# DevSinghSachan/emdr2

Measured on AMD Instinct MI355X. Metric: mips_queries_per_sec, higher is better.
Workload: dtype f16; 1 GPU; BASELINE configs[1]: MIPS-only top-50, 512 queries/search over a 21015324 x 768 fp16 index resident in HBM; rows=21015324, dim=768, top_k=50, parallelism=index row-sharded x1, all-gather(top-k) + merge, cus=256, allgather_bytes_per_rank=0

## Files before the change

### emdr2_amd/csrc/mips_api.hip

```cpp
#include "../../include/emdr2_mips.h"
#include "mips_kernels.h"
#include "exp_hooks.h"
#include <stdlib.h>

namespace {

#define TIMING_SLOTS 2048
struct Timing {
    bool enabled = false;
    hipEvent_t ev[2 * TIMING_SLOTS] = {};
    int created = 0;
    int n = 0;
    int64_t rows[TIMING_SLOTS] = {};
} g_timing;

int cu_count()
{
    static int cus = 0;
    if (!cus) {
        int dev = 0;
        hipDeviceProp_t prop;
        if (hipGetDevice(&dev) != hipSuccess || hipGetDeviceProperties(&prop, dev) != hipSuccess) return 256;
        cus = prop.multiProcessorCount > 0 ? prop.multiProcessorCount : 256;
    }
    return cus;
}

inline size_t align_up(size_t x, size_t a) { return (x + a - 1) / a * a; }

#define env_int(name, dflt) EXP_ENV_INT(name, dflt)

struct Workspace {
    char *q_frag;
    char *q_tiled;
    float *qnorm, *tau;
    unsigned *count;
    uint2 *cand, *cand8;
};

size_t carve(char *base, int dim, Workspace *w)
{
    size_t off = 0;
    auto take = [&](size_t bytes) { char *p = base ? base + off : nullptr; off += align_up(bytes, 256); return p; };
    char *f = take((size_t)(dim / 32) * 512 * 64);
    char *a = take((size_t)(dim / 32) * 512 * 64);
    char *b = take(512 * sizeof(float));
    char *c = take(512 * sizeof(float));
    char *d = take((512 + 8 * 512 + 8 * (size_t)SCAN8_PROG_UINTS) * sizeof(unsigned));
    char *e = take((size_t)512 * CAPQ * sizeof(uint2));
    char *g = take((size_t)512 * 8 * SUBCAP * sizeof(uint2));
    if (w) { w->q_frag = f; w->q_tiled = a; w->qnorm = (float *)b; w->tau = (float *)c; w->count = (unsigned *)d; w->cand = (uint2 *)e; w->cand8 = (uint2 *)g; }
    return off;
}

struct Shadow {
    const void *image;
    const float *table;
    int64_t min_rows;
};
long g_shadow_launches = 0;

bool bad_shape(int64_t n_rows, int dim) { return n_rows < 0 || n_rows >= ((int64_t)1 << 31) - 1024 || dim < 64 || dim > 8192 || (dim % 32) != 0; }

}

extern "C" {

int emdr2_abi_version(void) { return EMDR2_ABI_VERSION; }

int emdr2_device_cu_count(void) { return cu_count(); }

int emdr2_mips_set_timing(int enabled)
{
    g_timing.enabled = enabled != 0;
    g_timing.n = 0;
    return EMDR2_OK;
}

int emdr2_mips_timing_collect(float *ms, int64_t *rows, int max_n, int *n_out)
{
    const int n = g_timing.n < max_n ? g_timing.n : max_n;
    for (int i = 0; i < n; ++i) {
        if (hipEventSynchronize(g_timing.ev[2 * i + 1]) != hipSuccess) return EMDR2_E_LAUNCH;
        if (hipEventElapsedTime(&ms[i], g_timing.ev[2 * i], g_timing.ev[2 * i + 1]) != hipSuccess) return EMDR2_E_LAUNCH;
        rows[i] = g_timing.rows[i];
    }
    if (n_out) *n_out = n;
    g_timing.n = 0;
    return EMDR2_OK;
}

int emdr2_mips_layout_bytes(int64_t n_rows, int dim, size_t *bytes)
{
    if (!bytes || bad_shape(n_rows, dim)) return EMDR2_E_BADARG;
    const int64_t padded = (n_rows + 511) / 512 * 512;
    *bytes = (size_t)padded * dim * 2;
    return EMDR2_OK;
}

int emdr2_mips_pack_rows(const void *rows_rm, int64_t n_chunk, int dim, int64_t row_offset, int64_t n_rows_total,
                         void *tiled, float *emax_sq, emdr2_stream_t stream)
{
    if (!rows_rm || !tiled || !emax_sq || bad_shape(n_rows_total, dim) || n_chunk < 0 || row_offset < 0 ||
        row_offset + n_chunk > n_rows_total)
        return EMDR2_E_BADARG;
    return mips_launch_pack_rows(rows_rm, n_chunk, dim, row_offset, tiled, emax_sq, (hipStream_t)stream);
}

int emdr2_mips_unpack_rows(const void *tiled, int64_t n_rows_total, int dim, const int64_t *row_ids, int64_t n_out,
                           void *rows_rm, emdr2_stream_t stream)
{
    if (!tiled || !row_ids || !rows_rm || bad_shape(n_rows_total, dim) || n_out < 0) return EMDR2_E_BADARG;
    return mips_launch_unpack_rows(tiled, dim, row_ids, n_out, rows_rm, (hipStream_t)stream);
}

int emdr2_mips_workspace_bytes(int n_q, int dim, int k, size_t *bytes)
{
    if (!bytes || n_q < 1 || k < 1 || k > EMDR2_MAX_TOPK || bad_shape(0, dim)) return EMDR2_E_BADARG;
    *bytes = carve(nullptr, dim, nullptr);
    return EMDR2_OK;
}

static int variant_for(int nq) { return nq <= 128 ? 2 : (nq <= 256 ? 1 : 0); }
static const int kBM[3] = {128, 256, 512};
static const int kBN[3] = {512, 256, 128};

static int search_impl(const void *tiled, int64_t n_rows, int dim, int64_t row_base, const float *emax_sq,
                       const void *queries, int n_q, int k, const int32_t *ids, void *out_dist, int32_t *out_idx,
                       int64_t *out_row, uint32_t *out_flags, void *workspace, size_t workspace_bytes,
                       emdr2_stream_t stream_, int f32, uint4 *out_rec = nullptr, const Shadow *shadow = nullptr)
{
    if (!tiled || !emax_sq || !queries || !out_flags || !workspace) return EMDR2_E_BADARG;
    if (!out_rec && (!out_dist || !out_idx || !out_row)) return EMDR2_E_BADARG;
    if (out_rec && ((uintptr_t)out_rec & 15)) return EMDR2_E_BADARG;
    if (n_q < 1 || k < 1 || k > EMDR2_MAX_TOPK || bad_shape(n_rows, dim) || n_rows < 1) return EMDR2_E_BADARG;
    Workspace w;
    if (carve((char *)workspace, dim, &w) > workspace_bytes) return EMDR2_E_WORKSPACE;
    hipStream_t stream = (hipStream_t)stream_;
    const int kp = k <= 56 ? 64 : 128;
    const int seg0 = env_int("EMDR2_MIPS_SEG0", 8192) / 512 * 512;
    const int growth = env_int("EMDR2_MIPS_GROWTH", 8);
    const int growth_i8 = env_int("EMDR2_MIPS_GROWTH_I8", 2);
    if (seg0 < 512 || seg0 > (int)CAPQ - 512 || growth < 2 || growth_i8 < 2) return EMDR2_E_BADARG;
    const int force_variant = env_int("EMDR2_MIPS_VARIANT", -1);
    const int cus = env_int("EMDR2_MIPS_GRID", cu_count());
    const int scan_kernel = env_int("EMDR2_MIPS_KERNEL", 1);
    const int ablate = env_int("EMDR2_MIPS_ABLATE", 0);

    for (int q0 = 0; q0 < n_q; q0 += EMDR2_MAX_QUERIES_PER_PASS) {
        const int nqp = (n_q - q0) < EMDR2_MAX_QUERIES_PER_PASS ? (n_q - q0) : EMDR2_MAX_QUERIES_PER_PASS;
        int variant = variant_for(nqp);
        if (force_variant >= 0 && force_variant <= 2 && kBN[force_variant] >= nqp) variant = force_variant;
        const int BM = kBM[variant], BN = kBN[variant];
        const uint16_t *qp = (const uint16_t *)queries + (size_t)q0 * dim;
        int rc;
        if ((rc = mips_launch_pack_queries(qp, nqp, dim, BN, w.q_tiled, w.qnorm, stream))) return rc;
        EXP_MIPS_PACK_QUERIES_FRAG(variant, scan_kernel, qp, nqp, dim, w, stream, rc)
        const int64_t dense_rows = n_rows < seg0 ? n_rows : seg0;
        unsigned *const count8 = w.count + 512, *const prog0 = count8 + 8 * 512;
        if ((rc = mips_launch_init(w.tau, w.count, out_flags + q0, BN, nqp, (unsigned)dense_rows, count8,
                                   8 * 512 + (variant == 0 ? 8 * (size_t)SCAN8_PROG_UINTS : 0), stream)))
            return rc;

        ScanParams sp;
        sp.e_tiled = (const char *)tiled;
        sp.q_tiled = w.q_tiled;
        sp.tau = w.tau;
        sp.cand = w.cand;
        sp.count = w.count;
        sp.flags = out_flags + q0;
        sp.dense_out = nullptr;
        sp.nch = dim / 32;
        sp.n_rows = (int)n_rows;
        sp.n_q = nqp;
        sp.capq = CAPQ;
        sp.cand8 = w.cand8;
        sp.count8 = count8;
        sp.dense_row0 = 0;
        sp.tune = env_int("EMDR2_MIPS_TUNE", 17);
        sp.trace = (unsigned long long *)w.cand + (size_t)511 * CAPQ;

        int scan8_launches = 0;
        const bool shadow_ok = shadow && variant <= 1 && scan_kernel == 1 && (dim % 256) == 0 && n_rows - dense_rows >= shadow->min_rows;
        char *const q8_tiled = w.q_frag;
        float *const qc = (float *)(w.q_frag + (size_t)(dim / 64) * 512 * 64);
        if (shadow_ok && (rc = mips_launch_pack_queries_i8(qp, nqp, dim, BN, q8_tiled, qc, stream))) return rc;
        const bool couple = EXP_MIPS_COUPLE();
        int64_t done = 0, seg_end = dense_rows;
        int mode = 1;
        while (done < n_rows) {
            sp.tile_begin = (int)(done / BM);
            sp.tile_end = (int)((seg_end + BM - 1) / BM);
            const int tiles = sp.tile_end - sp.tile_begin;
            const int grid = tiles < cus ? tiles : cus;
            const bool timed = g_timing.enabled && g_timing.n < TIMING_SLOTS;
            if (timed) {
                while (g_timing.created <= g_timing.n) {
                    if (hipEventCreate(&g_timing.ev[2 * g_timing.created]) != hipSuccess ||
                        hipEventCreate(&g_timing.ev[2 * g_timing.created + 1]) != hipSuccess)
                        return EMDR2_E_LAUNCH;
                    ++g_timing.created;
                }
                if (hipEventRecord(g_timing.ev[2 * g_timing.n], stream) != hipSuccess) return EMDR2_E_LAUNCH;
            }
            bool int8_segment = false;
            EXP_MIPS_SCAN_VARIANT(mode, variant, ablate, scan_kernel, sp, w, grid, seg_end, n_rows, done, stream, rc)
            {
                rc = -4;
                if (mode == 0 && variant <= 1 && scan_kernel == 1) {
                    unsigned *prog = (couple && scan8_launches < 8) ? prog0 + (size_t)SCAN8_PROG_UINTS * scan8_launches : nullptr;
                    if (shadow_ok && seg_end - done >= shadow->min_rows) {
                        rc = mips_launch_scan8i(sp, shadow->image, shadow->table, q8_tiled, qc, BN, done, seg_end, cus, prog, stream);
                        if (rc == 0) { int8_segment = true; ++g_shadow_launches; }
                    }
                    if (rc == -4) rc = mips_launch_scan8(sp, BN, done, seg_end, cus, prog, stream);
                    if (rc == 0) ++scan8_launches;
                }
                if (rc == -4) rc = mips_launch_scan(variant, mode, sp, grid, stream);
            }
            if (rc) return rc;
            if (timed) {
                if (hipEventRecord(g_timing.ev[2 * g_timing.n + 1], stream) != hipSuccess) return EMDR2_E_LAUNCH;
                g_timing.rows[g_timing.n] = seg_end - done;
                ++g_timing.n;
            }
            if (int8_segment && (rc = mips_launch_rescore(sp, qp, (unsigned)kp, stream))) return rc;
            if (seg_end < n_rows && (rc = mips_launch_select(w.cand, w.count, w.cand8, count8, w.tau, out_flags + q0, CAPQ, kp, nqp, stream))) return rc;
            done = seg_end;
            const int64_t next_boundary = done * ((shadow_ok && done * (growth_i8 - 1) >= shadow->min_rows) ? growth_i8 : growth);
            seg_end = next_boundary < n_rows ? next_boundary : n_rows;
            if (n_rows - seg_end < seg_end / 2) seg_end = n_rows;
            mode = 0;
        }

        FinalizeParams fp;
        fp.e_tiled = (const char *)tiled;
        fp.queries = qp;
        fp.cand = w.cand;
        fp.count = w.count;
        fp.cand8 = w.cand8;
        fp.count8 = count8;
        fp.tau = w.tau;
        fp.qnorm = w.qnorm;
        fp.emax_sq = emax_sq;
        fp.ids = ids;
        fp.out_rec = out_rec ? out_rec + (size_t)q0 * k : nullptr;
        fp.out_dist = out_rec ? nullptr : (f32 ? (void *)((float *)out_dist + (size_t)q0 * k) : (void *)((uint16_t *)out_dist + (size_t)q0 * k));
        fp.f32 = f32;
        fp.out_idx = out_rec ? nullptr : out_idx + (size_t)q0 * k;
        fp.out_row = out_rec ? nullptr : out_row + (size_t)q0 * k;
        fp.flags = out_flags + q0;
        fp.n_rows = n_rows;
        fp.row_base = row_base;
        fp.dim = dim;
        fp.n_q = nqp;
        fp.k = k;
        fp.kp = kp;
        fp.capq = CAPQ;
        if ((rc = mips_launch_finalize(fp, true, stream))) return rc;
    }
    return EMDR2_OK;
}

int emdr2_mips_search(const void *tiled, int64_t n_rows, int dim, int64_t row_base, const float *emax_sq,
                      const void *queries, int n_q, int k, const int32_t *ids, void *out_dist, int32_t *out_idx,
                      int64_t *out_row, uint32_t *out_flags, void *workspace, size_t workspace_bytes,
                      emdr2_stream_t stream)
{
    return search_impl(tiled, n_rows, dim, row_base, emax_sq, queries, n_q, k, ids, out_dist, out_idx, out_row, out_flags, workspace,
                       workspace_bytes, stream, 0);
}

int emdr2_mips_search_f32(const void *tiled, int64_t n_rows, int dim, int64_t row_base, const float *emax_sq,
                          const void *queries, int n_q, int k, const int32_t *ids, float *out_dist, int32_t *out_idx,
                          int64_t *out_row, uint32_t *out_flags, void *workspace, size_t workspace_bytes,
                          emdr2_stream_t stream)
{
    return search_impl(tiled, n_rows, dim, row_base, emax_sq, queries, n_q, k, ids, out_dist, out_idx, out_row, out_flags, workspace,
                       workspace_bytes, stream, 1);
}

int emdr2_mips_search_records(const void *tiled, int64_t n_rows, int dim, int64_t row_base, const float *emax_sq, const void *queries, int n_q,
                              int k, const int32_t *ids, int f32, void *out_records, uint32_t *out_flags, void *workspace,
                              size_t workspace_bytes, emdr2_stream_t stream)
{
    if (!out_records) return EMDR2_E_BADARG;
    return search_impl(tiled, n_rows, dim, row_base, emax_sq, queries, n_q, k, ids, nullptr, nullptr, nullptr, out_flags, workspace,
                       workspace_bytes, stream, f32 ? 1 : 0, (uint4 *)out_records);
}

int emdr2_mips_shadow_bytes(int64_t n_rows, int dim, size_t *image_bytes, size_t *table_bytes)
{
    if (!image_bytes || !table_bytes || bad_shape(n_rows, dim) || (dim % 256) != 0) return EMDR2_E_BADARG;
    const int64_t padded = (n_rows + 511) / 512 * 512;
    *image_bytes = (size_t)padded * dim;
    *table_bytes = (size_t)(padded / 256) * 4 * sizeof(float);
    return EMDR2_OK;
}

int emdr2_mips_seal_shadow(const void *tiled, int64_t n_rows, int dim, void *shadow, void *table, uint32_t *nonfinite, emdr2_stream_t stream)
{
    if (!tiled || !shadow || !table || !nonfinite || ((uintptr_t)table & 15) || bad_shape(n_rows, dim) || (dim % 256) != 0) return EMDR2_E_BADARG;
    return mips_launch_seal_shadow(tiled, n_rows, dim, shadow, (float *)table, nonfinite, (hipStream_t)stream);
}

int emdr2_mips_search_shadow(const void *tiled, int64_t n_rows, int dim, int64_t row_base, const float *emax_sq, const void *shadow,
                             const void *table, int64_t shadow_min_rows, const void *queries, int n_q, int k, const int32_t *ids, int f32,
                             void *out_dist, int32_t *out_idx, int64_t *out_row, void *out_records, uint32_t *out_flags, void *workspace,
                             size_t workspace_bytes, emdr2_stream_t stream)
{
    if (!shadow || !table || ((uintptr_t)table & 15) || shadow_min_rows < 1 || (dim % 256) != 0) return EMDR2_E_BADARG;
    const Shadow sh = {shadow, (const float *)table, shadow_min_rows};
    return search_impl(tiled, n_rows, dim, row_base, emax_sq, queries, n_q, k, ids, out_dist, out_idx, out_row, out_flags, workspace,
                       workspace_bytes, stream, f32 ? 1 : 0, (uint4 *)out_records, &sh);
}

int emdr2_mips_shadow_launches(void) { return (int)g_shadow_launches; }

int emdr2_mips_merge_records(const void *records_in, int n_shards, int n_q, int k, int f32, void *out_dist, int32_t *out_idx, int64_t *out_row,
                             emdr2_stream_t stream)
{
    if (!records_in || ((uintptr_t)records_in & 15) || !out_dist || !out_idx || !out_row || n_shards < 1 || n_q < 1 || k < 1) return EMDR2_E_BADARG;
    return mips_launch_merge_records((const uint4 *)records_in, n_shards, n_q, k, f32 ? 1 : 0, out_dist, out_idx, out_row, (hipStream_t)stream);
}

int emdr2_mips_pack_records(const void *dist, const int32_t *idx, const int64_t *row, const int32_t *sel, int n_sel, int k, int f32,
                            void *records, emdr2_stream_t stream)
{
    if (!dist || !idx || !row || !sel || !records || ((uintptr_t)records & 15) || n_sel < 0 || k < 1) return EMDR2_E_BADARG;
    return mips_launch_pack_records(dist, idx, row, sel, n_sel, k, f32 ? 1 : 0, (uint4 *)records, (hipStream_t)stream);
}

int emdr2_mips_exact_workspace_bytes_f32(int64_t n_rows, int n_sel, size_t *bytes)
{
    if (!bytes || n_rows < 1 || n_sel < 0) return EMDR2_E_BADARG;
    *bytes = align_up((size_t)8 * (size_t)n_rows * sizeof(uint32_t), 256);
    return EMDR2_OK;
}

int emdr2_mips_search_exact_f32(const void *tiled, int64_t n_rows, int dim, int64_t row_base, const void *queries,
                                int n_q, const int32_t *sel, int n_sel, int k, const int32_t *ids, float *out_dist,
                                int32_t *out_idx, int64_t *out_row, uint32_t *out_flags, void *workspace,
                                size_t workspace_bytes, emdr2_stream_t stream_)
{
    if (!tiled || !queries || !sel || !out_dist || !out_idx || !out_row || !out_flags || !workspace) return EMDR2_E_BADARG;
    if (n_q < 1 || n_sel < 0 || k < 1 || k > EMDR2_MAX_TOPK || bad_shape(n_rows, dim) || n_rows < 1) return EMDR2_E_BADARG;
    if (workspace_bytes < (size_t)8 * (size_t)n_rows * sizeof(uint32_t)) return EMDR2_E_WORKSPACE;
    hipStream_t stream = (hipStream_t)stream_;
    for (int b = 0; b < n_sel; b += 8) {
        const int nb = (n_sel - b) < 8 ? (n_sel - b) : 8;
        int rc;
        if ((rc = mips_launch_exact_scores_f32((const char *)tiled, n_rows, dim, (const uint16_t *)queries, sel + b, nb,
                                               (uint32_t *)workspace, stream)))
            return rc;
        if ((rc = mips_launch_exact_select_f32((const uint32_t *)workspace, n_rows, row_base, sel + b, nb, k, ids, out_dist, out_idx,
                                               out_row, out_flags, stream)))
            return rc;
    }
    return EMDR2_OK;
}

int emdr2_mips_merge_f32(const float *dist_in, const int32_t *idx_in, const int64_t *row_in, int n_shards, int n_q, int k,
                         float *out_dist, int32_t *out_idx, int64_t *out_row, emdr2_stream_t stream)
{
    if (!dist_in || !idx_in || !row_in || !out_dist || !out_idx || !out_row || n_shards < 1 || n_q < 1 || k < 1) return EMDR2_E_BADARG;
    return mips_launch_merge_f32(dist_in, idx_in, row_in, n_shards, n_q, k, out_dist, out_idx, out_row, (hipStream_t)stream);
}

int emdr2_mips_exact_workspace_bytes(int64_t n_rows, int n_sel, size_t *bytes)
{
    if (!bytes || n_rows < 1 || n_sel < 0) return EMDR2_E_BADARG;
    *bytes = align_up((size_t)8 * (size_t)n_rows * sizeof(uint16_t), 256);
    return EMDR2_OK;
}

int emdr2_mips_search_exact(const void *tiled, int64_t n_rows, int dim, int64_t row_base, const void *queries,
                            int n_q, const int32_t *sel, int n_sel, int k, const int32_t *ids, void *out_dist,
                            int32_t *out_idx, int64_t *out_row, uint32_t *out_flags, void *workspace,
                            size_t workspace_bytes, emdr2_stream_t stream_)
{
    if (!tiled || !queries || !sel || !out_dist || !out_idx || !out_row || !out_flags || !workspace) return EMDR2_E_BADARG;
    if (n_q < 1 || n_sel < 0 || k < 1 || k > EMDR2_MAX_TOPK || bad_shape(n_rows, dim) || n_rows < 1) return EMDR2_E_BADARG;
    if (workspace_bytes < (size_t)8 * (size_t)n_rows * sizeof(uint16_t)) return EMDR2_E_WORKSPACE;
    hipStream_t stream = (hipStream_t)stream_;
    for (int b = 0; b < n_sel; b += 8) {
        const int nb = (n_sel - b) < 8 ? (n_sel - b) : 8;
        int rc;
        if ((rc = mips_launch_exact_scores((const char *)tiled, n_rows, dim, (const uint16_t *)queries, sel + b, nb,
                                           (uint16_t *)workspace, stream)))
            return rc;
        if ((rc = mips_launch_exact_select((const uint16_t *)workspace, n_rows, row_base, sel + b, nb, k, ids,
                                           (uint16_t *)out_dist, out_idx, out_row, out_flags, stream)))
            return rc;
    }
    return EMDR2_OK;
}

int emdr2_mips_merge(const void *dist_in, const int32_t *idx_in, const int64_t *row_in, int n_shards, int n_q, int k,
                     void *out_dist, int32_t *out_idx, int64_t *out_row, emdr2_stream_t stream)
{
    if (!dist_in || !idx_in || !row_in || !out_dist || !out_idx || !out_row || n_shards < 1 || n_q < 1 || k < 1) return EMDR2_E_BADARG;
    return mips_launch_merge((const uint16_t *)dist_in, idx_in, row_in, n_shards, n_q, k, (uint16_t *)out_dist, out_idx,
                             out_row, (hipStream_t)stream);
}

int emdr2_mips_debug_scores(const void *tiled, int64_t n_rows, int dim, const void *queries, int n_q,
                            float *out_scores, void *workspace, size_t workspace_bytes, emdr2_stream_t stream_)
{
    if (!tiled || !queries || !out_scores || !workspace || n_q < 1 || n_q > 512 || bad_shape(n_rows, dim) || n_rows < 1) return EMDR2_E_BADARG;
    Workspace w;
    if (carve((char *)workspace, dim, &w) > workspace_bytes) return EMDR2_E_WORKSPACE;
    hipStream_t stream = (hipStream_t)stream_;
    int variant = variant_for(n_q);
    const int force_variant = env_int("EMDR2_MIPS_VARIANT", -1);
    if (force_variant >= 0 && force_variant <= 2 && kBN[force_variant] >= n_q) variant = force_variant;
    const int BM = kBM[variant], BN = kBN[variant];
    int rc;
    if ((rc = mips_launch_pack_queries(queries, n_q, dim, BN, w.q_tiled, w.qnorm, stream))) return rc;
    ScanParams sp;
    sp.e_tiled = (const char *)tiled;
    sp.q_tiled = w.q_tiled;
    sp.tau = w.tau;
    sp.cand = w.cand;
    sp.count = w.count;
    sp.flags = nullptr;
    sp.dense_out = out_scores;
    sp.nch = dim / 32;
    sp.n_rows = (int)n_rows;
    sp.n_q = n_q;
    sp.capq = CAPQ;
    sp.cand8 = nullptr;
    sp.count8 = nullptr;
    sp.dense_row0 = 0;
    sp.tune = 1;
    sp.trace = nullptr;
    sp.tile_begin = 0;
    sp.tile_end = (int)((n_rows + BM - 1) / BM);
    const int cus = cu_count();
    return mips_launch_scan(variant, 2, sp, sp.tile_end < cus ? sp.tile_end : cus, stream);
}

}
```

### emdr2_amd/csrc/mips_kernels.h

```cpp
#pragma once
#include <hip/hip_runtime.h>
#include <stdint.h>

#define CAPQ 16384u
#define SUBCAP 1024u

struct ScanParams {
    const char *e_tiled;
    const char *q_tiled;
    const float *tau;
    uint2 *cand;
    unsigned *count;
    unsigned *flags;
    float *dense_out;
    int nch;
    int tile_begin, tile_end;
    int n_rows;
    int n_q;
    unsigned capq;
    uint2 *cand8;
    unsigned *count8;
    int dense_row0;
    int tune;
    unsigned long long *trace;
};

int mips_launch_scan(int variant, int mode, const ScanParams &p, int grid, hipStream_t stream);
#define SCAN8_PROG_UINTS (256 * 64)
int mips_launch_scan8(const ScanParams &p, int bn, int64_t row_begin, int64_t row_end, int cus, unsigned *prog, hipStream_t stream);
int mips_launch_seal_shadow(const void *tiled, int64_t n_rows, int dim, void *e8, float *blk, unsigned *nonfinite, hipStream_t stream);
int mips_launch_pack_queries_i8(const void *queries, int n_q, int dim, int bn, void *q8_tiled, float *qc, hipStream_t stream);
int mips_launch_scan8i(const ScanParams &p, const void *e8_tiled, const float *blk, const void *q8_tiled, const float *qc, int bn, int64_t row_begin,
                       int64_t row_end, int cus, unsigned *prog, hipStream_t stream);
int mips_launch_rescore(const ScanParams &p, const void *queries, unsigned pre, hipStream_t stream);
int mips_launch_scan_pp(int variant, int depth, const ScanParams &p, int grid, hipStream_t stream);
int mips_launch_scan_q8(int abl, const ScanParams &p, int grid, hipStream_t stream);
int mips_launch_pack_queries_frag(const void *queries, int n_q, int dim, void *q_frag, hipStream_t stream);
int mips_launch_scan_ablate(int abl, const ScanParams &p, int grid, hipStream_t stream);

int mips_launch_pack_rows(const void *rows_rm, int64_t n_chunk, int dim, int64_t row_offset, void *tiled,
                          float *emax_sq, hipStream_t stream);
int mips_launch_unpack_rows(const void *tiled, int dim, const int64_t *row_ids, int64_t n_out, void *rows_rm,
                            hipStream_t stream);
int mips_launch_pack_queries(const void *queries, int n_q, int dim, int bn, void *q_tiled, float *qnorm,
                             hipStream_t stream);
int mips_launch_init(float *tau, unsigned *count, unsigned *flags, int bn, int n_q, unsigned dense_count, unsigned *zero, size_t n_zero,
                     hipStream_t stream);
int mips_launch_select(uint2 *cand, unsigned *count, uint2 *cand8, unsigned *count8, float *tau, unsigned *flags, unsigned capq, int kp, int n_q,
                       hipStream_t stream);
struct FinalizeParams {
    const char *e_tiled;
    const uint16_t *queries;
    const uint2 *cand;
    const unsigned *count;
    uint2 *cand8;
    unsigned *count8;
    const float *tau;
    const float *qnorm;
    const float *emax_sq;
    const int32_t *ids;
    void *out_dist;
    int32_t *out_idx;
    int64_t *out_row;
    unsigned *flags;
    int64_t n_rows, row_base;
    int dim, n_q, k, kp;
    unsigned capq;
    int f32;
    uint4 *out_rec;
};
int mips_launch_finalize(const FinalizeParams &p, bool select_first, hipStream_t stream);
int mips_launch_merge_f32(const float *dist_in, const int32_t *idx_in, const int64_t *row_in, int n_shards, int n_q, int k,
                          float *out_dist, int32_t *out_idx, int64_t *out_row, hipStream_t stream);
int mips_launch_merge_records(const uint4 *rec_in, int n_shards, int n_q, int k, int f32, void *out_dist, int32_t *out_idx, int64_t *out_row,
                              hipStream_t stream);
int mips_launch_pack_records(const void *dist, const int32_t *idx, const int64_t *row, const int32_t *sel, int n_sel, int k, int f32, uint4 *rec,
                             hipStream_t stream);
int mips_launch_merge(const uint16_t *dist_in, const int32_t *idx_in, const int64_t *row_in, int n_shards, int n_q,
                      int k, uint16_t *out_dist, int32_t *out_idx, int64_t *out_row, hipStream_t stream);

int mips_launch_exact_scores(const char *e_tiled, int64_t n_rows, int dim, const uint16_t *queries,
                             const int32_t *sel, int n_sel, uint16_t *hkeys ,
                             hipStream_t stream);
int mips_launch_exact_select(const uint16_t *hkeys, int64_t n_rows, int64_t row_base, const int32_t *sel, int n_sel,
                             int k, const int32_t *ids, uint16_t *out_dist, int32_t *out_idx, int64_t *out_row,
                             unsigned *flags, hipStream_t stream);

int mips_launch_exact_scores_f32(const char *e_tiled, int64_t n_rows, int dim, const uint16_t *queries, const int32_t *sel, int n_sel,
                                 uint32_t *keys , hipStream_t stream);
int mips_launch_exact_select_f32(const uint32_t *keys, int64_t n_rows, int64_t row_base, const int32_t *sel, int n_sel, int k,
                                 const int32_t *ids, float *out_dist, int32_t *out_idx, int64_t *out_row, unsigned *flags, hipStream_t stream);
```

### emdr2_amd/csrc/mips_scan8i.hip

```cpp
#include "mips_scan8.h"

namespace {

typedef int intx4 __attribute__((ext_vector_type(4)));

struct Scan8iParams : Scan8Params {
    const float4 *blk;
    const float4 *qc;
};

__device__ __forceinline__ int s8i_theta(float tau, float t, float a, float b, float s, float n, float d)
{
    if (tau == __builtin_inff()) return 0x7fffffff;
    const float ts = t * s;
    if (!(ts > 0.f)) return (int)0x80000000;
    const float eps = (a * n + b * d) * 1.0001f;
    float num = tau - eps;
    num -= fabsf(num) * 1e-6f;
    float x = num * __builtin_amdgcn_rcpf(ts);
    x -= fabsf(x) * 1e-5f;
    x = floorf(x) - 1.f;
    if (!(x > -2.0e9f)) return (int)0x80000000;
    if (x > 2.0e9f) return 0x7fffffff;
    return (int)x;
}

struct Scan8Int8 {
    typedef Scan8iParams Params;
    typedef intx4 frag_t;
    typedef intx4 acc_t;
    typedef int val_t;
    typedef float4 QConst;
    struct ItemConst { float s, n, d; };
    static __device__ __forceinline__ acc_t mfma(frag_t a, frag_t b, acc_t c) { return __builtin_amdgcn_mfma_i32_16x16x64_i8(a, b, c, 0, 0, 0); }
    static __device__ __forceinline__ QConst load_q(const Params &P, int q) { return P.qc[q < P.s.n_q ? q : 0]; }
    static __device__ __forceinline__ ItemConst load_item(const Params &P, int tile)
    {
        const __attribute__((address_space(4))) float *bk = (const __attribute__((address_space(4))) float *)(uintptr_t)(P.blk + tile);
        return {bk[0], bk[1], bk[2]};
    }
    static __device__ __forceinline__ int threshold(float tau, const QConst &qc, const ItemConst &ic) { return s8i_theta(tau, qc.x, qc.y, qc.z, ic.s, ic.n, ic.d); }
    static __device__ __forceinline__ int max2(int a, int b) { return max(a, b); }
    static __device__ __forceinline__ unsigned bits(int v) { return (unsigned)v; }
};

}

namespace {

__device__ __forceinline__ float block_max_256(float v, float *sh)
{
#pragma unroll
    for (int o = 32; o >= 1; o >>= 1) v = fmaxf(v, __shfl_xor(v, o));
    __syncthreads();
    if ((threadIdx.x & 63) == 0) sh[threadIdx.x >> 6] = v;
    __syncthreads();
    return fmaxf(fmaxf(sh[0], sh[1]), fmaxf(sh[2], sh[3]));
}

__device__ __forceinline__ int quant8(float x, float inv)
{
    int v = (int)rintf(x * inv);
    return v > 127 ? 127 : (v < -127 ? -127 : v);
}

__global__ void __launch_bounds__(256) seal_shadow_kernel(const char *__restrict__ tiled, int nch, char *__restrict__ e8, float4 *__restrict__ blk,
                                                          unsigned *__restrict__ nonfinite)
{
    __shared__ float sh[4];
    const int64_t row = (int64_t)blockIdx.x * 256 + threadIdx.x;
    const int nseg = nch * 4;
    float amax = 0.f, n2 = 0.f;
    bool bad = false;
    for (int seg = 0; seg < nseg; ++seg) {
        const uint4 v = *(const uint4 *)(tiled + tiled_seg_offset(row, seg, nch));
        const half8 h = __builtin_bit_cast(half8, v);
#pragma unroll
        for (int j = 0; j < 8; ++j) {
            const float x = (float)h[j];
            bad |= !(fabsf(x) <= 65504.f);
            amax = fmaxf(amax, fabsf(x));
            n2 += x * x;
        }
    }
    if (bad) atomicOr(nonfinite, 1u);
    amax = block_max_256(amax, sh);
    n2 = block_max_256(n2, sh);
    const float s = amax / 127.f;
    const float inv = s > 0.f ? 127.f / amax : 0.f;
    float d2 = 0.f;
    const int nch8 = nch >> 1;
    for (int g = 0; g < nseg / 2; ++g) {
        unsigned w[4];
#pragma unroll
        for (int hf = 0; hf < 2; ++hf) {
            const uint4 v = *(const uint4 *)(tiled + tiled_seg_offset(row, 2 * g + hf, nch));
            const half8 h = __builtin_bit_cast(half8, v);
#pragma unroll
            for (int j = 0; j < 8; j += 4) {
                unsigned pk = 0;
#pragma unroll
                for (int b = 0; b < 4; ++b) {
                    const float x = (float)h[j + b];
                    const int qv = quant8(x, inv);
                    const float r = x - s * (float)qv;
                    d2 += r * r;
                    pk |= ((unsigned)qv & 255u) << (8 * b);
                }
                w[2 * hf + (j >> 2)] = pk;
            }
        }
        *(uint4 *)(e8 + tiled_seg_offset(row, g, nch8)) = make_uint4(w[0], w[1], w[2], w[3]);
    }
    d2 = block_max_256(d2, sh);
    const float nb = sqrtf(n2) * 1.001f;
    if (threadIdx.x == 0) blk[blockIdx.x] = make_float4(s, nb, (sqrtf(d2) + nb * 0x1p-22f) * 1.001f, 0.f);
}

__global__ void pack_queries_i8_kernel(const uint4 *__restrict__ queries, int n_q, int nseg, int bn, char *__restrict__ q8, float4 *__restrict__ qc)
{
    const int q = blockIdx.x, lane = threadIdx.x;
    float amax = 0.f;
    if (q < n_q)
        for (int seg = lane; seg < nseg; seg += 64) {
            const half8 h = __builtin_bit_cast(half8, queries[(size_t)q * nseg + seg]);
#pragma unroll
            for (int j = 0; j < 8; ++j) amax = fmaxf(amax, fabsf((float)h[j]));
        }
#pragma unroll
    for (int o = 32; o >= 1; o >>= 1) amax = fmaxf(amax, __shfl_xor(amax, o));
    const float t = amax / 127.f;
    const float inv = t > 0.f ? 127.f / amax : 0.f;
    float a2 = 0.f, b2 = 0.f;
    for (int g = lane; g < nseg / 2; g += 64) {
        unsigned w[4] = {0u, 0u, 0u, 0u};
        if (q < n_q) {
#pragma unroll
            for (int hf = 0; hf < 2; ++hf) {
                const half8 h = __builtin_bit_cast(half8, queries[(size_t)q * nseg + 2 * g + hf]);
#pragma unroll
                for (int j = 0; j < 8; ++j) {
                    const float x = (float)h[j];
                    const int qv = quant8(x, inv);
                    const float y = t * (float)qv, r = x - y;
                    a2 += r * r; b2 += y * y;
                    w[2 * hf + (j >> 2)] |= ((unsigned)qv & 255u) << (8 * (j & 3));
                }
            }
        }
        const int c = g >> 2, sp = (g & 3) ^ ((q >> 2) & 3);
        *(uint4 *)(q8 + ((size_t)c * bn * 4 + (size_t)q * 4 + sp) * 16) = make_uint4(w[0], w[1], w[2], w[3]);
    }
#pragma unroll
    for (int o = 32; o >= 1; o >>= 1) { a2 += __shfl_xor(a2, o); b2 += __shfl_xor(b2, o); }
    const float ra = sqrtf(a2), rb = sqrtf(b2);
    if (lane == 0) qc[q] = q < n_q ? make_float4(t, (ra + (ra + rb) * 0x1p-22f) * 1.001f, rb * 1.001f, 0.f) : make_float4(0.f, 0.f, 0.f, 0.f);
}

__global__ void __launch_bounds__(256) rescore_kernel(const char *__restrict__ tiled, const uint4 *__restrict__ queries, int nseg, uint2 *cand,
                                                      const unsigned *__restrict__ count, uint2 *cand8, const unsigned *__restrict__ count8,
                                                      unsigned capq, unsigned pre)
{
    const int q = blockIdx.y, list = blockIdx.x, lane = threadIdx.x & 63, wave = threadIdx.x >> 6;
    uint2 *ent;
    unsigned lo, hi;
    if (list < 8) {
        ent = cand8 + ((size_t)q * 8 + list) * SUBCAP; lo = 0; hi = count8[list * 512 + q];
        if (hi > SUBCAP) hi = SUBCAP;
    } else {
        ent = cand + (size_t)q * capq; lo = pre; hi = count[q];
        if (hi > capq) hi = capq;
    }
    const uint4 *qrow = queries + (size_t)q * nseg;
    const int nch = nseg >> 2;
    for (unsigned i0 = lo + 2 * wave; i0 < hi; i0 += 8) {
        const bool two = i0 + 1 < hi;
        const unsigned r0 = ent[i0].y, r1 = ent[two ? i0 + 1 : i0].y;
        float s0 = 0.f, s1 = 0.f;
        for (int seg = lane; seg < nseg; seg += 64) {
            const half8 e0 = __builtin_bit_cast(half8, *(const uint4 *)(tiled + tiled_seg_offset(r0, seg, nch)));
            const half8 e1 = __builtin_bit_cast(half8, *(const uint4 *)(tiled + tiled_seg_offset(r1, seg, nch)));
            const half8 qv = __builtin_bit_cast(half8, qrow[seg]);
#pragma unroll
            for (int j = 0; j < 8; ++j) { s0 += (float)e0[j] * (float)qv[j]; s1 += (float)e1[j] * (float)qv[j]; }
        }
#pragma unroll
        for (int o = 32; o >= 1; o >>= 1) { s0 += __shfl_xor(s0, o); s1 += __shfl_xor(s1, o); }
        if (lane == 0) {
            ent[i0].x = __float_as_uint(s0);
            if (two) ent[i0 + 1].x = __float_as_uint(s1);
        }
    }
}

}

int mips_launch_seal_shadow(const void *tiled, int64_t n_rows, int dim, void *e8, float *blk, unsigned *nonfinite, hipStream_t stream)
{
    const int64_t blocks = (n_rows + 255) / 256;
    if (blocks == 0) return 0;
    hipLaunchKernelGGL(seal_shadow_kernel, dim3((unsigned)blocks), dim3(256), 0, stream, (const char *)tiled, dim / 32, (char *)e8, (float4 *)blk, nonfinite);
    return hipGetLastError() == hipSuccess ? 0 : -3;
}

int mips_launch_pack_queries_i8(const void *queries, int n_q, int dim, int bn, void *q8_tiled, float *qc, hipStream_t stream)
{
    hipLaunchKernelGGL(pack_queries_i8_kernel, dim3(bn), dim3(64), 0, stream, (const uint4 *)queries, n_q, dim / 8, bn, (char *)q8_tiled, (float4 *)qc);
    return hipGetLastError() == hipSuccess ? 0 : -3;
}

int mips_launch_rescore(const ScanParams &p, const void *queries, unsigned pre, hipStream_t stream)
{
    hipLaunchKernelGGL(rescore_kernel, dim3(9, p.n_q), dim3(256), 0, stream, p.e_tiled, (const uint4 *)queries, p.nch * 4, p.cand, p.count, p.cand8,
                       p.count8, p.capq, pre);
    return hipGetLastError() == hipSuccess ? 0 : -3;
}

int mips_launch_scan8i(const ScanParams &p, const void *e8_tiled, const float *blk, const void *q8_tiled, const float *qc, int bn, int64_t row_begin,
                       int64_t row_end, int cus, unsigned *prog, hipStream_t stream)
{
    if (p.nch & 7) return -4;
    Scan8iParams P;
    P.s = p;
    P.s.e_tiled = (const char *)e8_tiled;
    P.s.q_tiled = (const char *)q8_tiled;
    P.s.nch = p.nch / 2;
    P.blk = (const float4 *)blk;
    P.qc = (const float4 *)qc;
    return s8_launch<Scan8Int8>(P, bn, row_begin, row_end, cus, prog, stream);
}
```

Before: 60550 queries/s.

## Defer exact rescoring of int8 candidates unlikely to beat threshold

Replaces the per-segment exact fp16 rescore of int8-scan candidates with a triage kernel. The triage computes an error-bounded estimate and rescoring happens right away only for candidates whose estimate plus a margin reaches the current threshold. The others are parked in a pending buffer with their upper bound and rescored after the last select, only if that bound still beats the final tau. The rescore inner loop is also widened to four rows per wave. The aim is to avoid fp16 gathers for most int8 candidates, at the cost of an extra select launch, a new workspace buffer and overflow handling when PENDCAP fills.

```diff
diff --git a/emdr2_amd/csrc/mips_api.hip b/emdr2_amd/csrc/mips_api.hip
--- a/emdr2_amd/csrc/mips_api.hip
+++ b/emdr2_amd/csrc/mips_api.hip
@@ -35,7 +35,7 @@
     char *q_tiled;
     float *qnorm, *tau;
     unsigned *count;
-    uint2 *cand, *cand8;
+    uint2 *cand, *cand8, *pend;
 };
 
 size_t carve(char *base, int dim, Workspace *w)
@@ -46,10 +46,11 @@
     char *a = take((size_t)(dim / 32) * 512 * 64);
     char *b = take(512 * sizeof(float));
     char *c = take(512 * sizeof(float));
-    char *d = take((512 + 8 * 512 + 8 * (size_t)SCAN8_PROG_UINTS) * sizeof(unsigned));
+    char *d = take((512 + 8 * 512 + 512 + 8 * (size_t)SCAN8_PROG_UINTS) * sizeof(unsigned));
     char *e = take((size_t)512 * CAPQ * sizeof(uint2));
     char *g = take((size_t)512 * 8 * SUBCAP * sizeof(uint2));
-    if (w) { w->q_frag = f; w->q_tiled = a; w->qnorm = (float *)b; w->tau = (float *)c; w->count = (unsigned *)d; w->cand = (uint2 *)e; w->cand8 = (uint2 *)g; }
+    char *h = take((size_t)512 * PENDCAP * sizeof(uint2));
+    if (w) { w->q_frag = f; w->q_tiled = a; w->qnorm = (float *)b; w->tau = (float *)c; w->count = (unsigned *)d; w->cand = (uint2 *)e; w->cand8 = (uint2 *)g; w->pend = (uint2 *)h; }
     return off;
 }
 
@@ -141,6 +142,7 @@
     const int seg0 = env_int("EMDR2_MIPS_SEG0", 8192) / 512 * 512;
     const int growth = env_int("EMDR2_MIPS_GROWTH", 8);
     const int growth_i8 = env_int("EMDR2_MIPS_GROWTH_I8", 2);
+    const float margin_i8 = (float)env_int("EMDR2_MIPS_MARGIN_PCT", 25) * 0.01f;
     if (seg0 < 512 || seg0 > (int)CAPQ - 512 || growth < 2 || growth_i8 < 2) return EMDR2_E_BADARG;
     const int force_variant = env_int("EMDR2_MIPS_VARIANT", -1);
     const int cus = env_int("EMDR2_MIPS_GRID", cu_count());
@@ -157,9 +159,9 @@
         if ((rc = mips_launch_pack_queries(qp, nqp, dim, BN, w.q_tiled, w.qnorm, stream))) return rc;
         EXP_MIPS_PACK_QUERIES_FRAG(variant, scan_kernel, qp, nqp, dim, w, stream, rc)
         const int64_t dense_rows = n_rows < seg0 ? n_rows : seg0;
-        unsigned *const count8 = w.count + 512, *const prog0 = count8 + 8 * 512;
+        unsigned *const count8 = w.count + 512, *const pcount = count8 + 8 * 512, *const prog0 = pcount + 512;
         if ((rc = mips_launch_init(w.tau, w.count, out_flags + q0, BN, nqp, (unsigned)dense_rows, count8,
-                                   8 * 512 + (variant == 0 ? 8 * (size_t)SCAN8_PROG_UINTS : 0), stream)))
+                                   9 * 512 + (variant == 0 ? 8 * (size_t)SCAN8_PROG_UINTS : 0), stream)))
             return rc;
 
         ScanParams sp;
@@ -188,6 +190,7 @@
         const bool couple = EXP_MIPS_COUPLE();
         int64_t done = 0, seg_end = dense_rows;
         int mode = 1;
+        bool pending = false;
         while (done < n_rows) {
             sp.tile_begin = (int)(done / BM);
             sp.tile_end = (int)((seg_end + BM - 1) / BM);
@@ -224,8 +227,14 @@
                 g_timing.rows[g_timing.n] = seg_end - done;
                 ++g_timing.n;
             }
-            if (int8_segment && (rc = mips_launch_rescore(sp, qp, (unsigned)kp, stream))) return rc;
-            if (seg_end < n_rows && (rc = mips_launch_select(w.cand, w.count, w.cand8, count8, w.tau, out_flags + q0, CAPQ, kp, nqp, stream))) return rc;
+            if (int8_segment) {
+                if ((rc = mips_launch_triage(sp, qp, (unsigned)kp, shadow->table, qc, w.pend, pcount, margin_i8, stream))) return rc;
+                pending = true;
+            }
+            if ((seg_end < n_rows || pending) &&
+                (rc = mips_launch_select(w.cand, w.count, w.cand8, count8, w.tau, out_flags + q0, CAPQ, kp, nqp, stream)))
+                return rc;
+            if (seg_end >= n_rows && pending && (rc = mips_launch_rescore_pending(sp, qp, w.pend, pcount, stream))) return rc;
             done = seg_end;
             const int64_t next_boundary = done * ((shadow_ok && done * (growth_i8 - 1) >= shadow->min_rows) ? growth_i8 : growth);
             seg_end = next_boundary < n_rows ? next_boundary : n_rows;
diff --git a/emdr2_amd/csrc/mips_kernels.h b/emdr2_amd/csrc/mips_kernels.h
--- a/emdr2_amd/csrc/mips_kernels.h
+++ b/emdr2_amd/csrc/mips_kernels.h
@@ -4,6 +4,7 @@
 
 #define CAPQ 16384u
 #define SUBCAP 1024u
+#define PENDCAP 8192u
 
 struct ScanParams {
     const char *e_tiled;
@@ -32,7 +33,9 @@
 int mips_launch_pack_queries_i8(const void *queries, int n_q, int dim, int bn, void *q8_tiled, float *qc, hipStream_t stream);
 int mips_launch_scan8i(const ScanParams &p, const void *e8_tiled, const float *blk, const void *q8_tiled, const float *qc, int bn, int64_t row_begin,
                        int64_t row_end, int cus, unsigned *prog, hipStream_t stream);
-int mips_launch_rescore(const ScanParams &p, const void *queries, unsigned pre, hipStream_t stream);
+int mips_launch_triage(const ScanParams &p, const void *queries, unsigned pre, const float *blk, const float *qc, void *pend, unsigned *pcount,
+                       float margin, hipStream_t stream);
+int mips_launch_rescore_pending(const ScanParams &p, const void *queries, const void *pend, const unsigned *pcount, hipStream_t stream);
 int mips_launch_scan_pp(int variant, int depth, const ScanParams &p, int grid, hipStream_t stream);
 int mips_launch_scan_q8(int abl, const ScanParams &p, int grid, hipStream_t stream);
 int mips_launch_pack_queries_frag(const void *queries, int n_q, int dim, void *q_frag, hipStream_t stream);
diff --git a/emdr2_amd/csrc/mips_scan8i.hip b/emdr2_amd/csrc/mips_scan8i.hip
--- a/emdr2_amd/csrc/mips_scan8i.hip
+++ b/emdr2_amd/csrc/mips_scan8i.hip
@@ -23,6 +23,18 @@
     if (!(x > -2.0e9f)) return (int)0x80000000;
     if (x > 2.0e9f) return 0x7fffffff;
     return (int)x;
+}
+
+struct S8iBound { float est, eps, upper; };
+__device__ __forceinline__ S8iBound s8i_upper(int isum, float t, float a, float b, float s, float n, float d, float dim)
+{
+    S8iBound r;
+    r.est = t * s * (float)isum;
+    r.eps = (a * n + b * d) * 1.0001f;
+    const float slack = dim * 0x1p-22f * (a + b) * n * 1.0001f;
+    const float u = r.est + fabsf(r.est) * 1e-6f + r.eps + slack;
+    r.upper = u + fabsf(u) * 1e-6f;
+    return r;
 }
 
 struct Scan8Int8 {
@@ -157,11 +169,73 @@
     if (lane == 0) qc[q] = q < n_q ? make_float4(t, (ra + (ra + rb) * 0x1p-22f) * 1.001f, rb * 1.001f, 0.f) : make_float4(0.f, 0.f, 0.f, 0.f);
 }
 
-__global__ void __launch_bounds__(256) rescore_kernel(const char *__restrict__ tiled, const uint4 *__restrict__ queries, int nseg, uint2 *cand,
-                                                      const unsigned *__restrict__ count, uint2 *cand8, const unsigned *__restrict__ count8,
-                                                      unsigned capq, unsigned pre)
-{
-    const int q = blockIdx.y, list = blockIdx.x, lane = threadIdx.x & 63, wave = threadIdx.x >> 6;
+__device__ __forceinline__ void rescore_wave_x4(const char *__restrict__ tiled, const unsigned (&rows)[4], const uint4 *__restrict__ qrow, int nseg, int lane,
+                                                float (&out)[4])
+{
+    const int nch = nseg >> 2;
+    float s[4] = {0.f, 0.f, 0.f, 0.f};
+    for (int seg = lane; seg < nseg; seg += 64) {
+        uint4 ev[4];
+#pragma unroll
+        for (int c = 0; c < 4; ++c) ev[c] = *(const uint4 *)(tiled + tiled_seg_offset(rows[c], seg, nch));
+        const half8 qv = __builtin_bit_cast(half8, qrow[seg]);
+#pragma unroll
+        for (int c = 0; c < 4; ++c) {
+            const half8 e = __builtin_bit_cast(half8, ev[c]);
+#pragma unroll
+            for (int j = 0; j < 8; ++j) s[c] += (float)e[j] * (float)qv[j];
+        }
+    }
+#pragma unroll
+    for (int o = 32; o >= 1; o >>= 1)
+#pragma unroll
+        for (int c = 0; c < 4; ++c) s[c] += __shfl_xor(s[c], o);
+#pragma unroll
+    for (int c = 0; c < 4; ++c) out[c] = s[c];
+}
+
+__device__ __forceinline__ unsigned block_rank_256(bool flag, unsigned *sh, unsigned &total)
+{
+    const int lane = threadIdx.x & 63, wave = threadIdx.x >> 6;
+    const unsigned long long m = __builtin_amdgcn_ballot_w64(flag);
+    const unsigned before = __builtin_amdgcn_mbcnt_hi((unsigned)(m >> 32), __builtin_amdgcn_mbcnt_lo((unsigned)m, 0));
+    __syncthreads();
+    if (lane == 0) sh[wave] = (unsigned)__popcll(m);
+    __syncthreads();
+    unsigned off = 0, tot = 0;
+#pragma unroll
+    for (int w = 0; w < 4; ++w) { const unsigned v = sh[w]; off += w < wave ? v : 0u; tot += v; }
+    total = tot;
+    return off + before;
+}
+
+__device__ __forceinline__ void rescore_worklist(const char *__restrict__ tiled, const uint4 *__restrict__ qrow, int nseg, const unsigned *sh_row,
+                                                 const unsigned *sh_idx, unsigned n, uint2 *dst, unsigned dst_end)
+{
+    const int lane = threadIdx.x & 63, wave = threadIdx.x >> 6;
+    for (unsigned j0 = 4 * wave; j0 < n; j0 += 16) {
+        unsigned rows[4];
+#pragma unroll
+        for (int c = 0; c < 4; ++c) rows[c] = sh_row[j0 + c < n ? j0 + c : j0];
+        float sc[4];
+        rescore_wave_x4(tiled, rows, qrow, nseg, lane, sc);
+#pragma unroll
+        for (int c = 0; c < 4; ++c)
+            if (lane == 0 && j0 + c < n) {
+                const unsigned i = sh_idx[j0 + c];
+                if (i < dst_end) dst[i] = make_uint2(__float_as_uint(sc[c]), rows[c]);
+            }
+    }
+}
+
+__global__ void __launch_bounds__(256) triage_kernel(const char *__restrict__ tiled, const uint4 *__restrict__ queries, int nseg, uint2 *cand,
+                                                     const unsigned *__restrict__ count, uint2 *cand8, const unsigned *__restrict__ count8, unsigned capq,
+                                                     unsigned pre, const float4 *__restrict__ blk, const float4 *__restrict__ qc,
+                                                     const float *__restrict__ tau, uint2 *pend, unsigned *pcount, float margin)
+{
+    __shared__ unsigned long long sh_def[CAPQ / 64];
+    __shared__ unsigned sh4[4], sh_base, sh_row[256], sh_idx[256];
+    const int q = blockIdx.y, list = blockIdx.x, tid = threadIdx.x;
     uint2 *ent;
     unsigned lo, hi;
     if (list < 8) {
@@ -170,26 +244,84 @@
     } else {
         ent = cand + (size_t)q * capq; lo = pre; hi = count[q];
         if (hi > capq) hi = capq;
-    }
+        if (hi > CAPQ) hi = CAPQ;
+    }
+    if (lo >= hi) return;
+    const float4 c = qc[q];
+    const float tq = tau[q], dimf = (float)(nseg * 8);
+    uint2 *const pq = pend + (size_t)q * PENDCAP;
+    auto deferred = [&](unsigned i, uint2 &e, float &upper) {
+        e = ent[i];
+        const float4 b = blk[e.y >> 8];
+        const S8iBound r = s8i_upper((int)e.x, c.x, c.y, c.z, b.x, b.y, b.z, dimf);
+        upper = r.upper;
+        return !(r.est + margin * r.eps >= tq);
+    };
+    unsigned mine = 0;
+    for (unsigned i0 = lo; i0 < hi; i0 += 256) {
+        const unsigned i = i0 + tid;
+        uint2 e; float u;
+        const unsigned long long m = __builtin_amdgcn_ballot_w64(i < hi && deferred(i, e, u));
+        if ((tid & 63) == 0) { sh_def[((i0 - lo) >> 6) + (tid >> 6)] = m; mine += (unsigned)__popcll(m); }
+    }
+    if ((tid & 63) == 0) sh4[tid >> 6] = mine;
+    __syncthreads();
+    if (tid == 0) {
+        const unsigned total = sh4[0] + sh4[1] + sh4[2] + sh4[3];
+        sh_base = total ? atomicAdd(&pcount[q], total) : 0u;
+    }
+    __syncthreads();
+    unsigned next = sh_base;
     const uint4 *qrow = queries + (size_t)q * nseg;
-    const int nch = nseg >> 2;
-    for (unsigned i0 = lo + 2 * wave; i0 < hi; i0 += 8) {
-        const bool two = i0 + 1 < hi;
-        const unsigned r0 = ent[i0].y, r1 = ent[two ? i0 + 1 : i0].y;
-        float s0 = 0.f, s1 = 0.f;
-        for (int seg = lane; seg < nseg; seg += 64) {
-            const half8 e0 = __builtin_bit_cast(half8, *(const uint4 *)(tiled + tiled_seg_offset(r0, seg, nch)));
-            const half8 e1 = __builtin_bit_cast(half8, *(const uint4 *)(tiled + tiled_seg_offset(r1, seg, nch)));
-            const half8 qv = __builtin_bit_cast(half8, qrow[seg]);
-#pragma unroll
-            for (int j = 0; j < 8; ++j) { s0 += (float)e0[j] * (float)qv[j]; s1 += (float)e1[j] * (float)qv[j]; }
-        }
-#pragma unroll
-        for (int o = 32; o >= 1; o >>= 1) { s0 += __shfl_xor(s0, o); s1 += __shfl_xor(s1, o); }
-        if (lane == 0) {
-            ent[i0].x = __float_as_uint(s0);
-            if (two) ent[i0 + 1].x = __float_as_uint(s1);
-        }
+    for (unsigned i0 = lo; i0 < hi; i0 += 256) {
+        const unsigned i = i0 + tid;
+        uint2 e = make_uint2(0u, 0u);
+        float u = 0.f;
+        if (i < hi) deferred(i, e, u);
+        const bool def = (sh_def[((i0 - lo) >> 6) + (tid >> 6)] >> (tid & 63)) & 1ull;
+        unsigned n_def;
+        const unsigned slot = next + block_rank_256(def, sh4, n_def);
+        next += n_def;
+        const bool parked = def && slot < PENDCAP;
+        if (parked) {
+            pq[slot] = make_uint2(__float_as_uint(u), e.y);
+            ent[i].x = 0xff800000u;
+        }
+        unsigned n_now;
+        const unsigned w = block_rank_256(i < hi && !parked, sh4, n_now);
+        if (i < hi && !parked) { sh_row[w] = e.y; sh_idx[w] = i; }
+        __syncthreads();
+        rescore_worklist(tiled, qrow, nseg, sh_row, sh_idx, n_now, ent, hi);
+    }
+}
+
+__global__ void __launch_bounds__(256) rescore_pending_kernel(const char *__restrict__ tiled, const uint4 *__restrict__ queries, int nseg, uint2 *cand,
+                                                              unsigned *count, unsigned capq, const float *__restrict__ tau, const uint2 *__restrict__ pend,
+                                                              const unsigned *__restrict__ pcount)
+{
+    __shared__ unsigned sh4[4], sh_base, sh_row[256], sh_idx[256];
+    const int q = blockIdx.y, tid = threadIdx.x;
+    unsigned np = pcount[q];
+    if (np > PENDCAP) np = PENDCAP;
+    const unsigned lo = (unsigned)((uint64_t)np * blockIdx.x / gridDim.x), hi = (unsigned)((uint64_t)np * (blockIdx.x + 1) / gridDim.x);
+    if (lo >= hi) return;
+    const float tq = tau[q];
+    const uint2 *const pq = pend + (size_t)q * PENDCAP;
+    const uint4 *qrow = queries + (size_t)q * nseg;
+    uint2 *const main_list = cand + (size_t)q * capq;
+    for (unsigned i0 = lo; i0 < hi; i0 += 256) {
+        const unsigned i = i0 + tid;
+        const uint2 e = i < hi ? pq[i] : make_uint2(0u, 0u);
+        const bool keep = i < hi && !(__uint_as_float(e.x) < tq);
+        unsigned n_keep;
+        const unsigned w = block_rank_256(keep, sh4, n_keep);
+        if (n_keep == 0) continue;
+        if (tid == 0) sh_base = atomicAdd(&count[q], n_keep);
+        if (keep) sh_row[w] = e.y;
+        __syncthreads();
+        if (keep) sh_idx[w] = sh_base + w;
+        __syncthreads();
+        rescore_worklist(tiled, qrow, nseg, sh_row, sh_idx, n_keep, main_list, capq);
     }
 }
 
@@ -209,10 +341,18 @@
     return hipGetLastError() == hipSuccess ? 0 : -3;
 }
 
-int mips_launch_rescore(const ScanParams &p, const void *queries, unsigned pre, hipStream_t stream)
-{
-    hipLaunchKernelGGL(rescore_kernel, dim3(9, p.n_q), dim3(256), 0, stream, p.e_tiled, (const uint4 *)queries, p.nch * 4, p.cand, p.count, p.cand8,
-                       p.count8, p.capq, pre);
+int mips_launch_triage(const ScanParams &p, const void *queries, unsigned pre, const float *blk, const float *qc, void *pend, unsigned *pcount,
+                       float margin, hipStream_t stream)
+{
+    hipLaunchKernelGGL(triage_kernel, dim3(9, p.n_q), dim3(256), 0, stream, p.e_tiled, (const uint4 *)queries, p.nch * 4, p.cand, p.count, p.cand8,
+                       p.count8, p.capq, pre, (const float4 *)blk, (const float4 *)qc, p.tau, (uint2 *)pend, pcount, margin);
+    return hipGetLastError() == hipSuccess ? 0 : -3;
+}
+
+int mips_launch_rescore_pending(const ScanParams &p, const void *queries, const void *pend, const unsigned *pcount, hipStream_t stream)
+{
+    hipLaunchKernelGGL(rescore_pending_kernel, dim3(8, p.n_q), dim3(256), 0, stream, p.e_tiled, (const uint4 *)queries, p.nch * 4, p.cand, p.count,
+                       p.capq, p.tau, (const uint2 *)pend, pcount);
     return hipGetLastError() == hipSuccess ? 0 : -3;
 }
 
```

After: 63310 queries/s (median of 6 runs). +4.6%, better.
